# mlvlab/BLiM

Hardware: AMD Instinct MI355X
Metric: candidate-pairs/sec (7B, 96+32 tok) (higher is better)
Workload: dtype f16; 1 GPU; SYN v2t-VTG re-rank: Qwen2-7B dims (28 layers), seeded synthetic weights, 96 video + 32 text tokens per pair, top-16 text candidates per video query, 55 queries (880 pairs, 32560 packed tokens, 28160 label rows) per step per GPU; prefix_reuse=True, vtg_compensated=none, parallelism=query rows sharded over 1 GPU(s); RCCL all-gather of score rows at the end

## Files before the change

blim_amd/csrc/gemm.hip:

```cpp
#include "gemm.hpp"
#include "kernels.hpp"
#include <type_traits>

#define BM 256
#define BN 256
#define BK 64
#define NTHREADS 512
#define TILE_BYTES (BM * BK * 2)
#define BUF_BYTES (2 * TILE_BYTES)
#define GROUP_M 8

typedef const __attribute__((address_space(1))) void* gptr_t;
typedef __attribute__((address_space(3))) void* lptr_t;

__device__ __forceinline__ void glds16(const void* g, char* lds_wave_base) {
    __builtin_amdgcn_global_load_lds((gptr_t)g, (lptr_t)lds_wave_base, 16, 0, 0);
}

__device__ __forceinline__ float gelu_erf(float x) {
    const float z = fabsf(x) * 0.70710678118654752f;
    const float t = __builtin_amdgcn_rcpf(fmaf(0.3275911f, z, 1.0f));
    const float poly = t * fmaf(t, fmaf(t, fmaf(t, fmaf(t, 1.061405429f, -1.453152027f), 1.421413741f), -0.284496736f), 0.254829592f);
    const float erf_abs = 1.0f - poly * __expf(-z * z);
    return 0.5f * x * (1.0f + copysignf(erf_abs, x));
}
__device__ __forceinline__ float silu_f(float x) { return x * __builtin_amdgcn_rcpf(1.0f + __expf(-x)); }

template <int EPI, int DT, bool SPLIT = false, bool MXA = false>
__global__ __launch_bounds__(NTHREADS) void gemm_kernel(const GemmParams p) {
    __shared__ __attribute__((aligned(16))) char smem[5 * TILE_BYTES];

    constexpr bool LO6_BF16_FENCE = MXA && DT == DT_BF16;
    const int tid = threadIdx.x;
    const int lane = tid & 63;
    const int wave = __builtin_amdgcn_readfirstlane(tid >> 6);
    const int wm = wave >> 2, wn = wave & 3;
    int stamp_vb = blockIdx.x;
    auto stamp = [&](int k) __attribute__((always_inline)) {
        if (p.debug_stamps && tid == 0) p.debug_stamps[(size_t)stamp_vb * 8 + k] = __builtin_amdgcn_s_memrealtime();
    };
    const int ntm = (p.M + BM - 1) / BM, ntn = (p.N + BN - 1) / BN;
    const int nwg = ntm * ntn;
#pragma unroll 1
    for (int vb = blockIdx.x; vb < (p.tile_map ? ((nwg + 255) & ~255) : nwg); vb += gridDim.x) {
    int pid;
    if (p.tile_map) {
        const int xcd = vb & 7, k = vb >> 3;
        pid = ((k >> 5) * 8 + xcd) * 32 + (k & 31);
        if (pid >= nwg) continue;
    } else {
        const int bid = vb, xcd = bid & 7, q = nwg >> 3, r = nwg & 7;
        pid = (xcd < r ? xcd * (q + 1) : r * (q + 1) + (xcd - r) * q) + (bid >> 3);
    }
    stamp_vb = pid;
    stamp(0);
    if constexpr (out16<DT>::value == DT_F16 || (LO6_BF16_FENCE)) { if (p.f16_saturate) f16_saturate_off(); }
    const int width = p.group_m * ntn;
    const int first_m = (pid / width) * p.group_m;
    const int gsz = min(ntm - first_m, p.group_m);
    const int tm = first_m + (pid % width) % gsz;
    const int tn = (pid % width) / gsz;
    const int row0 = tm * BM, col0 = tn * BN;

    const int sr = lane >> 3;
    const char* baseA = (const char*)p.A;
    const char* baseW = (const char*)p.W;

    constexpr int ES = (DT == DT_F8) ? 1 : 2;
    constexpr bool MX8 = MXA && DT == DT_F8;
    constexpr bool LO6 = MXA && DT != DT_F8;
    constexpr int ODT = out16<DT>::value;
    const int fr = lane & 15, fc = lane >> 4;
    const int fg = (fr >> 1) & 7;
    const int frag_off = (fr >> 3) * 1024 + (fr & 7) * 128 + 16 * ((fc ^ (fg & 3)) + 4 * (fg >> 2));
    const int a_off = (16 * wm) * 1024 + frag_off;
    const int b_off = (8 * wn) * 1024 + frag_off;

    f32x4 acc[8][4];
#pragma unroll
    for (int i = 0; i < 8; ++i)
#pragma unroll
        for (int j = 0; j < 4; ++j) acc[i][j] = (f32x4){0.f, 0.f, 0.f, 0.f};

    const int nk = p.K * ES / (BK * 2);
    const int nk6 = LO6 ? p.K6 / 128 : 0;
    float f8_scale = 0.f;
    if constexpr (DT == DT_F8) f8_scale = tid < 256 ? (p.row_scale ? p.row_scale[min(row0 + tid, p.M - 1)] : 1.0f) : p.col_scale[min(col0 + tid - 256, p.N - 1)];
    stamp(1);
    {
        const int grp = wave >> 2;
        typedef int i32x8 __attribute__((ext_vector_type(8)));
        typedef int i32x4 __attribute__((ext_vector_type(4)));
        bf16x8 fa[2][8], fb[2][4];
        i32x8 fa8[8], fb8[4];
        auto load_frags = [&](int offA_tile, int offB_tile) __attribute__((always_inline)) {
            const char* ba[2] = {smem + (offA_tile + a_off), smem + ((offA_tile + a_off) ^ 64)};
            const char* bb[2] = {smem + (offB_tile + b_off), smem + ((offB_tile + b_off) ^ 64)};
            if constexpr (DT == DT_F8) {
                auto rd = [](const char* q0, const char* q1) __attribute__((always_inline)) {
                    const i32x4 l = *(const i32x4*)q0, h = *(const i32x4*)q1;
                    return (i32x8){l[0], l[1], l[2], l[3], h[0], h[1], h[2], h[3]};
                };
#pragma unroll
                for (int ni = 0; ni < 4; ++ni) fb8[ni] = rd(bb[0] + ni * 2048, bb[1] + ni * 2048);
#pragma unroll
                for (int mi = 0; mi < 8; ++mi) fa8[mi] = rd(ba[0] + mi * 2048, ba[1] + mi * 2048);
            } else {
#pragma unroll
                for (int ks = 0; ks < 2; ++ks) {
#pragma unroll
                    for (int ni = 0; ni < 4; ++ni) fb[ks][ni] = *(const bf16x8*)(bb[ks] + ni * 2048);
#pragma unroll
                    for (int mi = 0; mi < 8; ++mi) fa[ks][mi] = *(const bf16x8*)(ba[ks] + mi * 2048);
                }
            }
        };
        uint2 mx_cur = make_uint2(0x7f7f7f7fu, 0x7f7f7f7fu), mx_nxt = mx_cur;
        const uint8_t* mx_base = nullptr;
        if constexpr (MX8) {
            int frm = fr;
            asm volatile("" : "+v"(frm));
            mx_base = p.a_mx + (int64_t)tm * 256 + (wm * 16 + frm) * 8;
        }
        auto mx_request = [&](int kt) __attribute__((always_inline)) {
            if constexpr (MX8) mx_nxt = *(const uint2*)(mx_base + (int64_t)min(kt, nk - 1) * p.mx_stride);
        };
        auto compute = [&]() __attribute__((always_inline)) {
            __builtin_amdgcn_s_setprio(1);
            if constexpr (DT == DT_F8) {
#define F8_ROW(MI)                                                                                                                                  \
                _Pragma("unroll") for (int ni = 0; ni < 4; ++ni)                                                                                    \
                    acc[MI][ni] = __builtin_amdgcn_mfma_scale_f32_16x16x128_f8f6f4(fb8[ni], fa8[MI], acc[MI][ni], 0, 0, 0, 0x7f7f7f7f, (MX8 ? (MI & 3) : 0), \
                                                                                  (int)(MX8 ? ((MI) < 4 ? mx_cur.x : mx_cur.y) : 0x7f7f7f7fu));
                F8_ROW(0) F8_ROW(1) F8_ROW(2) F8_ROW(3) F8_ROW(4) F8_ROW(5) F8_ROW(6) F8_ROW(7)
#undef F8_ROW
            } else {
#pragma unroll
                for (int ks = 0; ks < 2; ++ks)
#pragma unroll
                    for (int mi = 0; mi < 8; ++mi)
#pragma unroll
                        for (int ni = 0; ni < 4; ++ni)
                            acc[mi][ni] = mfma16<DT>(fb[ks][ni], fa[ks][mi], acc[mi][ni]);
            }
// ... 966 lines not shown
    if constexpr (ODT == DT_F16) { if (p.f16_saturate) f16_saturate_off(); }

    const int wrow0 = row0 + 32 * wm, wcol0 = col0 + 32 * wn;
    const int tq = lane >> 4, rsub = lane & 15;
    const bool rotated = wcol0 < p.rope_cols;
    float4 qkv_bias[2];
#pragma unroll
    for (int ni = 0; ni < 2; ++ni) {
        const int col = wcol0 + 16 * ni + 4 * tq;
        qkv_bias[ni] = col + 3 < p.N ? *(const float4*)(p.bias + col) : make_float4(0.f, 0.f, 0.f, 0.f);
    }
    const int g = (wcol0 & 127) >> 5;
    float4 cs[2], sn[2];
#pragma unroll
    for (int mi = 0; mi < 2; ++mi) cs[mi] = sn[mi] = make_float4(0.f, 0.f, 0.f, 0.f);
    if (rotated) {
        const int64_t cstride = p.rope_stride * 16;
#pragma unroll
        for (int mi = 0; mi < 2; ++mi) {
            const int row = min(wrow0 + 16 * mi + rsub, p.M - 1);
            const float* base = p.rope_rows + (int64_t)row * 16 + 4 * tq;
            cs[mi] = *(const float4*)(base + g * cstride);
            sn[mi] = *(const float4*)(base + (4 + g) * cstride);
        }
    }

    const NarrowAcc walked = narrow_walk<DT, LO6>(p, tm, tn, lane, wave);
    const f32x4 (&acc)[2][2] = walked.v;

    if constexpr (ODT == DT_F16) { if (p.f16_saturate) f16_saturate_on(); }
    auto ST = [&](int row, int col, float a_, float b_, float c_, float d_) __attribute__((always_inline)) {
        const uint2 hi_ = make_uint2(pack2<ODT>(a_, b_), pack2<ODT>(c_, d_));
        uint2 lo_ = make_uint2(0u, 0u);
        if constexpr (SPLIT) {
            const uint16_t* h16_ = (const uint16_t*)&hi_;
            lo_ = make_uint2(pack2<ODT>(a_ - from16<ODT>(h16_[0]), b_ - from16<ODT>(h16_[1])), pack2<ODT>(c_ - from16<ODT>(h16_[2]), d_ - from16<ODT>(h16_[3])));
        }
        if (row >= p.M || col + 3 >= p.N) return;
        bf16_t* out = (bf16_t*)p.C + (int64_t)row * p.ldc + col;
        *(uint2*)out = hi_;
        if constexpr (SPLIT) *(uint2*)(out + p.lo_off) = lo_;
    };
    if (rotated) {
        const int ncol = (wcol0 & ~127) + 16 * g + 4 * tq;
#pragma unroll
        for (int mi = 0; mi < 2; ++mi) {
            const int row = wrow0 + 16 * mi + rsub;
            const float4 c = cs[mi], sv = sn[mi];
            const float c4[4] = {c.x, c.y, c.z, c.w}, s4[4] = {sv.x, sv.y, sv.z, sv.w};
            const float4 b0 = qkv_bias[0], b1 = qkv_bias[1];
            const float bl[4] = {b0.x, b0.y, b0.z, b0.w}, bh[4] = {b1.x, b1.y, b1.z, b1.w};
            float lo[4], hi[4];
#pragma unroll
            for (int j = 0; j < 4; ++j) {
                const float x1 = acc[mi][0][j] + bl[j];
                const float x2 = acc[mi][1][j] + bh[j];
                lo[j] = __builtin_fmaf(x1, c4[j], -__fmul_rn(x2, s4[j]));
                hi[j] = __builtin_fmaf(x2, c4[j], __fmul_rn(x1, s4[j]));
            }
            ST(row, ncol, lo[0], lo[1], lo[2], lo[3]);
            ST(row, ncol + 64, hi[0], hi[1], hi[2], hi[3]);
        }
    } else {
#pragma unroll
        for (int mi = 0; mi < 2; ++mi) {
            const int row = wrow0 + 16 * mi + rsub;
#pragma unroll
            for (int ni = 0; ni < 2; ++ni) {
                const float4 bv = qkv_bias[ni];
                ST(row, wcol0 + 16 * ni + 4 * tq, acc[mi][ni][0] + bv.x, acc[mi][ni][1] + bv.y, acc[mi][ni][2] + bv.z, acc[mi][ni][3] + bv.w);
            }
        }
    }
}

#include <stdlib.h>
#include <algorithm>
#include <atomic>
static int g_gemm_skip_epi = getenv("BLIM_GEMM_SKIP_EPI") ? atoi(getenv("BLIM_GEMM_SKIP_EPI")) : 0;
static unsigned long long* g_gemm_stamps = nullptr;
static int g_stamp_epi = getenv("BLIM_GEMM_STAMP_EPI") ? atoi(getenv("BLIM_GEMM_STAMP_EPI")) : -1;
static int g_stamp_k = getenv("BLIM_GEMM_STAMP_K") ? atoi(getenv("BLIM_GEMM_STAMP_K")) : -1;
void gemm_set_debug_stamps(unsigned long long* buf) { g_gemm_stamps = buf; }

template <int EPI>
static int launch_t(const GemmParams& p, hipStream_t stream) {
    const int ntm = (p.M + BM - 1) / BM, ntn = (p.N + BN - 1) / BN;
    static int n_cu = 0;
    if (n_cu == 0) {
        int dev = 0;
        if (hipGetDevice(&dev) != hipSuccess || hipDeviceGetAttribute(&n_cu, hipDeviceAttributeMultiprocessorCount, dev) != hipSuccess || n_cu <= 0) n_cu = 256;
        n_cu = (n_cu / 8) * 8;
        if (n_cu < 8) n_cu = 8;
    }
    const dim3 grid(ntm * ntn < n_cu ? ntm * ntn : n_cu);
    void (*kernel)(const GemmParams) = nullptr;
    if constexpr (EPI == EPI_QKV || EPI == EPI_SWIGLU || EPI == EPI_RESID || EPI == EPI_LSE) {
        if (p.A6) {
#define LO6_KERNEL(DTX)                                                                                    \
            if constexpr (EPI == EPI_RESID || EPI == EPI_LSE) kernel = gemm_kernel<EPI, DTX, false, true>; \
            else if (p.lo_off != 0) kernel = gemm_kernel<EPI, DTX, true, true>;                            \
            else if constexpr (EPI == EPI_SWIGLU) kernel = gemm_kernel<EPI, DTX, false, true>;             \
            else { blim_set_error("lo6 QKV GEMM: hi | lo outputs only"); return BLIM_ERR_ARG; }
            if (p.dtype == DT_F16) { LO6_KERNEL(DT_F16) } else { LO6_KERNEL(DT_BF16) }
#undef LO6_KERNEL
        }
    }
    if constexpr (EPI == EPI_BF16 || EPI == EPI_QKV || EPI == EPI_SWIGLU) {
        if (!kernel && p.lo_off != 0) {
            if (p.dtype == DT_F16) kernel = gemm_kernel<EPI, DT_F16, true>;
            else if (p.dtype == DT_BF16) kernel = gemm_kernel<EPI, DT_BF16, true>;
            else { blim_set_error("split (hi|lo) GEMM outputs need a 16-bit engine"); return BLIM_ERR_ARG; }
        }
    }
    if constexpr (EPI == EPI_RESID) {
        if (!kernel && p.dtype == DT_F8 && p.a_mx) kernel = gemm_kernel<EPI, DT_F8, false, true>;
    }
    if (!kernel) {
        if (p.dtype == DT_F8) kernel = gemm_kernel<EPI, DT_F8>;
        else if (p.dtype == DT_F16) kernel = gemm_kernel<EPI, DT_F16>;
        else kernel = gemm_kernel<EPI, DT_BF16>;
    }
    hipLaunchKernelGGL(kernel, grid, dim3(NTHREADS), 0, stream, p);
    hipError_t e = hipGetLastError();
    if (e != hipSuccess) {
        blim_set_error("gemm launch failed: %s", hipGetErrorString(e));
        return BLIM_ERR_HIP;
    }
    return BLIM_OK;
}

static int launch_one(GemmEpi epi, const GemmParams& p_in, hipStream_t stream);

static bool narrow_eligible(GemmEpi epi, const GemmParams& p) {
    return epi == EPI_RESID && (p.dtype == DT_F16 || p.dtype == DT_BF16) && !p.A6 && !p.W6 && !p.a_mx && !p.swiglu_act && !p.debug_stamps && !p.debug_skip_epilogue;
}
static bool narrow_lo6_eligible(GemmEpi epi, const GemmParams& p) {
    return epi == EPI_RESID && (p.dtype == DT_F16 || p.dtype == DT_BF16) && p.A6 && p.W6 && p.w_wrap_k == 0 && !p.a_mx && !p.swiglu_act && !p.debug_stamps && !p.debug_skip_epilogue;
}
static bool narrow_qkv_eligible(GemmEpi epi, const GemmParams& p) {
    return epi == EPI_QKV && (p.dtype == DT_F16 || p.dtype == DT_BF16) && !(p.A6 && p.lo_off == 0) && p.lo_off % 4 == 0 && !p.a_mx && !p.debug_stamps && !p.debug_skip_epilogue;
}
#define NARROW_LAUNCH(...) hipLaunchKernelGGL((__VA_ARGS__), grid, dim3(N_THREADS), 0, stream, p)
static void launch_narrow(const GemmParams& p, dim3 grid, hipStream_t stream) {
    if (p.dtype == DT_F16) NARROW_LAUNCH(gemm_narrow_kernel<DT_F16>); else NARROW_LAUNCH(gemm_narrow_kernel<DT_BF16>);
}
static void launch_narrow_lo6(const GemmParams& p, dim3 grid, hipStream_t stream) {
    if (p.dtype == DT_F16) NARROW_LAUNCH(gemm_narrow_lo6_kernel<DT_F16>); else NARROW_LAUNCH(gemm_narrow_lo6_kernel<DT_BF16>);
}
template <int DT>
static void launch_narrow_qkv_t(const GemmParams& p, dim3 grid, hipStream_t stream) {
    if (p.A6) NARROW_LAUNCH(gemm_nqkv_kernel<DT, true, true>);
    else if (p.lo_off != 0) NARROW_LAUNCH(gemm_nqkv_kernel<DT, true, false>);
    else NARROW_LAUNCH(gemm_nqkv_kernel<DT, false, false>);
}
static void launch_narrow_qkv(const GemmParams& p, dim3 grid, hipStream_t stream) {
    if (p.dtype == DT_F16) launch_narrow_qkv_t<DT_F16>(p, grid, stream); else launch_narrow_qkv_t<DT_BF16>(p, grid, stream);
}
#undef NARROW_LAUNCH
struct NarrowForm {
    int GemmParams::*field;
    const char* name;
    const char* kernel;
    const char* tag;
    bool (*eligible)(GemmEpi, const GemmParams&);
    int threshold;
    void (*launch)(const GemmParams&, dim3, hipStream_t);
    std::atomic<int64_t> launches;
};
static NarrowForm g_narrow_forms[3] = {
    {&GemmParams::narrow, "narrow", "the narrow kernel", "narrow", narrow_eligible, GEMM_NARROW_TILES, launch_narrow, {0}},
    {&GemmParams::narrow_lo6, "narrow_lo6", "the narrow e2m3 kernel", "narrow lo6", narrow_lo6_eligible, GEMM_NARROW_LO6_TILES, launch_narrow_lo6, {0}},
    {&GemmParams::narrow_qkv, "narrow_qkv", "the narrow QKV kernel", "narrow qkv", narrow_qkv_eligible, GEMM_NARROW_QKV_TILES, launch_narrow_qkv, {0}},
};
extern "C" int64_t blim_gemm_narrow_launches(void) { return g_narrow_forms[0].launches.load(); }
extern "C" int32_t blim_gemm_narrow_threshold(void) { return g_narrow_forms[0].threshold; }
extern "C" int64_t blim_gemm_narrow_lo6_launches(void) { return g_narrow_forms[1].launches.load(); }
extern "C" int32_t blim_gemm_narrow_lo6_threshold(void) { return g_narrow_forms[1].threshold; }
extern "C" int64_t blim_gemm_narrow_qkv_launches(void) { return g_narrow_forms[2].launches.load(); }
extern "C" int32_t blim_gemm_narrow_qkv_threshold(void) { return g_narrow_forms[2].threshold; }
static NarrowForm* narrow_chosen(GemmEpi epi, const GemmParams& p) {
    for (NarrowForm& f : g_narrow_forms) {
        const int v = p.*f.field;
        if (v == 0 || !f.eligible(epi, p)) continue;
        if (v == 2 || (int64_t)((p.M + BM - 1) / BM) * ((p.N + BN - 1) / BN) < f.threshold) return &f;
    }
    return nullptr;
}
static int launch_narrow_form(NarrowForm& f, const GemmParams& p, hipStream_t stream) {
    f.launch(p, dim3((unsigned)(((p.M + NBM - 1) / NBM) * ((p.N + NBN - 1) / NBN))), stream);
    hipError_t e = hipGetLastError();
    if (e != hipSuccess) { blim_set_error("%s gemm launch failed: %s", f.tag, hipGetErrorString(e)); return BLIM_ERR_HIP; }
    f.launches.fetch_add(1);
    return BLIM_OK;
}

int launch_gemm(GemmEpi epi, const GemmParams& p, hipStream_t stream) {
    ARG_CHECK(p.M > 0 && p.N > 0 && p.K > 0 && p.lda > 0);
    ARG_CHECK(p.dtype == DT_BF16 || p.dtype == DT_F16 || p.dtype == DT_F8);
    const int64_t es = p.dtype == DT_F8 ? 1 : 2;
    const int64_t row_bytes = p.lda * es;
    if ((int64_t)p.M * row_bytes < (1ll << 32)) return launch_one(epi, p, stream);
    const int64_t chunk = ((1ll << 32) - 1) / row_bytes / BM * BM;
    ARG_CHECK(chunk >= BM);
    const int64_t c_es = (epi == EPI_F32 || epi == EPI_RESID) ? 4 : 2;
    const int ntn = (p.N + BN - 1) / BN;
    for (int64_t r0 = 0; r0 < p.M; r0 += chunk) {
        GemmParams q = p;
        q.M = (int)std::min<int64_t>(chunk, p.M - r0);
        q.A = (const bf16_t*)((const char*)p.A + r0 * row_bytes);
        if (p.C) q.C = (char*)p.C + r0 * p.ldc * c_es;
        if (p.row_scale) q.row_scale = p.row_scale + r0;
        if (p.rope_rows) q.rope_rows = p.rope_rows + r0 * 16;
        if (p.a_mx) q.a_mx = p.a_mx + r0;
        if (p.out_mx) q.out_mx = p.out_mx + r0;
        if (p.A6) q.A6 = p.A6 + (r0 / BM) * (int64_t)(p.K6 / 128) * F6_TILE_BYTES;
        if (p.out6) q.out6 = p.out6 + (r0 / BM) * (int64_t)(p.N / BN) * F6_TILE_BYTES;
        if (p.labels) q.labels = p.labels + r0;
        if (p.lse_part) q.lse_part = p.lse_part + r0 * ntn;
        if (p.label_logit) q.label_logit = p.label_logit + r0;
        if (p.resid_in) q.resid_in = p.resid_in + r0 * p.ldc;
        if (p.swiglu_gu) q.swiglu_gu = p.swiglu_gu + r0 * p.swiglu_ld;
        if (p.swiglu_act) q.swiglu_act = p.swiglu_act + r0 * p.swiglu_act_ld;
        const int rc = launch_one(epi, q, stream);
        if (rc != BLIM_OK) return rc;
    }
    return BLIM_OK;
}

static int launch_one(GemmEpi epi, const GemmParams& p_in, hipStream_t stream) {
    GemmParams p = p_in;
    p.debug_skip_epilogue = g_gemm_skip_epi;
    p.group_m = GROUP_M;
    const int64_t n_tiles = (int64_t)((p.M + BM - 1) / BM) * ((p.N + BN - 1) / BN);
    p.tile_map = ((p.N + BN - 1) / BN <= 32 && n_tiles >= 256) ? 1 : 0;
    p.debug_stamps = ((g_stamp_epi < 0 || g_stamp_epi == (int)epi) && (g_stamp_k < 0 || g_stamp_k == p.K)) ? g_gemm_stamps : nullptr;
    ARG_CHECK(p.M > 0 && p.N > 0 && p.K > 0);
    ARG_CHECK(p.A && p.W);
    ARG_CHECK(p.dtype == DT_BF16 || p.dtype == DT_F16 || p.dtype == DT_F8);
    const int es = p.dtype == DT_F8 ? 1 : 2;
    ARG_CHECK((int64_t)p.K * es % 128 == 0);
    ARG_CHECK(p.lda * es % 16 == 0);
    ARG_CHECK(p.dtype != DT_F8 || ((p.row_scale || p.a_mx) && p.col_scale));
    ARG_CHECK((!p.a_mx && !p.out_mx) || (p.dtype == DT_F8 && p.mx_stride >= (int64_t)((p.M + BM - 1) / BM) * 256));
    ARG_CHECK(!p.a_mx || epi == EPI_RESID);
    ARG_CHECK(!p.A6 || ((p.dtype == DT_F16 || p.dtype == DT_BF16) && p.W6 && p.w_wrap_k == 0 && p.K6 > 0 && p.K6 % 128 == 0 && (epi == EPI_RESID || epi == EPI_QKV || epi == EPI_SWIGLU || epi == EPI_LSE)));
    ARG_CHECK(!p.out_mx || (epi == EPI_SWIGLU && p.N % 256 == 0 && p.ldc % 16 == 0));
    ARG_CHECK(!p.out6 || (epi == EPI_SWIGLU && p.A6 && p.lo_off > 0 && p.N % 256 == 0));
    ARG_CHECK(p.w_wrap_k == 0 || (p.K == 2 * p.w_wrap_k && (int64_t)p.w_wrap_k * es % 128 == 0));
    ARG_CHECK(p.lo_off == 0 || epi == EPI_BF16 || epi == EPI_QKV || epi == EPI_SWIGLU);
    for (const NarrowForm& f : g_narrow_forms)
        if (p.*f.field < 0 || p.*f.field > 2) { blim_set_error("gemm: %s = %d (0 = the 256 x 256 kernel, 1 = auto, 2 = %s wherever it is eligible)", f.name, p.*f.field, f.kernel); return BLIM_ERR_ARG; }
    ARG_CHECK((int64_t)p.M * p.lda * es < (1ll << 32) && (int64_t)p.N * (p.w_wrap_k > 0 ? p.w_wrap_k : p.K) * es < (1ll << 32));
    switch (epi) {
        case EPI_BF16:
            ARG_CHECK(p.C && p.ldc % 4 == 0);
            ARG_CHECK(!p.swiglu_gu || (p.N % 16 == 0 && p.swiglu_ld % 8 == 0 && p.swiglu_ld >= 2 * (int64_t)p.N));
            ARG_CHECK(!p.swiglu_act || (p.N % 32 == 0 && p.swiglu_act_ld % 8 == 0 && p.swiglu_act_ld >= p.N / 2 && !p.swiglu_gu));
            return launch_t<EPI_BF16>(p, stream);
        case EPI_F32: ARG_CHECK(p.C && p.bias == nullptr); return launch_t<EPI_F32>(p, stream);
        case EPI_RESID:
            ARG_CHECK(p.C && p.ldc % 4 == 0);
            if (NarrowForm* f = narrow_chosen(epi, p)) return launch_narrow_form(*f, p, stream);
            return launch_t<EPI_RESID>(p, stream);
        case EPI_QKV:
            ARG_CHECK(p.C && p.bias && p.rope_rows && p.rope_stride >= p.M && p.N % 128 == 0 && p.rope_cols % 128 == 0 && p.ldc % 4 == 0);
            if (NarrowForm* f = narrow_chosen(epi, p)) return launch_narrow_form(*f, p, stream);
            return launch_t<EPI_QKV>(p, stream);
        case EPI_SWIGLU: ARG_CHECK(p.C && p.N % 32 == 0 && p.ldc % 4 == 0); return launch_t<EPI_SWIGLU>(p, stream);
        case EPI_LSE: ARG_CHECK(p.labels && p.lse_part && p.label_logit); return launch_t<EPI_LSE>(p, stream);
    }
    blim_set_error("unknown epilogue %d", (int)epi);
    return BLIM_ERR_ARG;
}
```

blim_amd/csrc/gemm.hpp:

```cpp
#pragma once
#include "common.hpp"

enum GemmEpi : int {
    EPI_BF16 = 0,
    EPI_F32 = 1,
    EPI_RESID = 2,
    EPI_QKV = 3,
    EPI_SWIGLU = 4,
    EPI_LSE = 5,
};

struct GemmParams {
    int dtype;
    const float* row_scale;
    const float* col_scale;
    const bf16_t* A;
    int64_t lda;
    const bf16_t* W;
    int M, N, K;
    void* C;
    int64_t ldc;
    const float* bias;
    const float* resid_in;
    uint16_t* swiglu_gu;
    int64_t swiglu_ld;
    uint16_t* swiglu_act;
    int64_t swiglu_act_ld;
    int act;
    float scale;
    int rope_cols;
    const float* rope_rows;
    int64_t rope_stride;
    const int32_t* labels;
    float2* lse_part;
    float* label_logit;
    int w_wrap_k;
    int64_t lo_off;
    uint8_t* out_mx;
    const uint8_t* a_mx;
    int64_t mx_stride;
    const uint8_t* A6;
    const uint8_t* W6;
    int K6;
    uint8_t* out6;
    int f16_saturate;
    int group_m;
    int tile_map;
    int debug_skip_epilogue;
    unsigned long long* debug_stamps;
    int narrow;
    int narrow_lo6;
    int narrow_qkv;
};
#define GEMM_NARROW_TILES 57
#define GEMM_NARROW_LO6_TILES 57
#define GEMM_NARROW_QKV_TILES 55
void gemm_set_debug_stamps(unsigned long long* buf);

int launch_gemm(GemmEpi epi, const GemmParams& p, hipStream_t stream);

static inline int qkv_perm_row(int cprime) { return 16 * (cprime >> 5) + (cprime & 15) + 64 * ((cprime >> 4) & 1); }
```

blim_amd/engine.py:

```python
from __future__ import annotations

import ctypes as C
import os
import re
from typing import Dict, List, Optional, Sequence

import numpy as np

from .synth import ModelDims, weight_shapes

_HERE = os.path.dirname(os.path.abspath(__file__))
LIB_PATH = os.environ.get("BLIM_LIB_PATH") or os.path.join(_HERE, "libblim_hip.so")
HEADER_PATH = os.path.join(os.path.dirname(_HERE), "include", "blim.h")

DTYPE_F32, DTYPE_BF16 = 0, 1
COMPUTE_DTYPES = {"bf16": 0, "f16": 1, "f8": 2}
DEFAULT_COMPUTE_DTYPE = os.environ.get("BLIM_DTYPE", "f16")


def torch_dtype_of(name: str):
    import torch
    return {"bf16": torch.bfloat16, "f16": torch.float16, "f8": torch.float16}[name]


# ... 103 lines not shown
    vp, i32, i64, u64, f32 = C.c_void_p, C.c_int32, C.c_int64, C.c_uint64, C.c_float
    sig = {
        "blim_abi_version": ([], C.c_int),
        "blim_last_error": ([], C.c_char_p),
        "blim_create": ([C.POINTER(Config), C.POINTER(vp)], C.c_int),
        "blim_destroy": ([vp], None),
        "blim_load_weight": ([vp, C.c_char_p, vp, i32, i32], C.c_int),
        "blim_init_synthetic_weights": ([vp, u64], C.c_int),
        "blim_weights_ready": ([vp], C.c_int),
        "blim_load_adapter": ([vp, C.c_char_p, vp, vp, i32, f32], C.c_int),
        "blim_clear_adapters": ([vp], C.c_int),
        "blim_num_adapters": ([vp], C.c_int),
        "blim_reserve": ([vp, i64, i64], C.c_int),
        "blim_project_video": ([vp, vp, i64, i32, vp, vp], C.c_int),
        "blim_group_mean": ([vp, vp, i64, i32, vp, vp], C.c_int),
        "blim_assemble": ([vp, vp, i64, vp, vp, vp], C.c_int),
        "blim_decode": ([vp, C.POINTER(Batch), vp, vp, i64, vp, vp, vp], C.c_int),
        "blim_vtg_logprobs": ([vp, vp, vp, i64, vp, vp], C.c_int),
        "blim_segment_mean": ([vp, vp, vp, i32, i32, vp, vp], C.c_int),
        "blim_lm_head": ([vp, vp, i64, vp, vp], C.c_int),
        "blim_ce_rows": ([vp, vp, i64, i32, vp, i64, vp, vp], C.c_int),
        "blim_visual_head": ([vp, vp, i64, vp, vp], C.c_int),
        "blim_visual_head_f32": ([vp, vp, i64, vp, vp], C.c_int),
        "blim_tvg_scores": ([vp, vp, vp, i32, vp, i32, vp, vp], C.c_int),
        "blim_tvg_logits": ([vp, vp, vp, i32, i32, vp, vp], C.c_int),
        "blim_set_video_vocab": ([vp, vp, i32, vp], C.c_int),
        "blim_tvg_logits_f32": ([vp, vp, i32, vp, vp], C.c_int),
        "blim_score_vtg": ([vp, C.POINTER(Batch), vp, vp, vp, i64, vp, i32, vp, vp], C.c_int),
        "blim_score_tvg": ([vp, C.POINTER(Batch), vp, vp, vp, i32, vp, i32, vp, vp], C.c_int),
        "blim_forward": ([vp, vp, vp, i32, i32, vp, vp, vp], C.c_int),
        "blim_fill_bell_bf16": ([vp, i64, u64, C.c_char_p, f32, f32, vp], C.c_int),
        "blim_fill_bell_f32": ([vp, i64, u64, C.c_char_p, f32, f32, i32, vp], C.c_int),
        "blim_gemm_bf16": ([vp, i64, vp, i32, i32, i32, vp, i64, vp], C.c_int),
        "blim_gemm_f16": ([vp, i64, vp, i32, i32, i32, vp, i64, vp], C.c_int),
        "blim_f6_tiles_bytes": ([i64, i32], C.c_int64),
        "blim_gemm_f16_lo6": ([vp, vp, i32, i32, i32, vp, vp, vp, vp], C.c_int),
        "blim_quant_rows": ([vp, i64, i64, i32, i32, vp, vp, vp], C.c_int),
        "blim_gemm_f8": ([vp, i64, vp, vp, vp, i32, i32, i32, vp, i64, vp], C.c_int),
        "blim_attention": ([C.POINTER(AttentionArgs), vp], C.c_int),
        "blim_attention_bwd_workspace_bytes": ([i64, i32, i32, i32], C.c_int64),
        "blim_attention_bwd": ([C.POINTER(AttentionBwdArgs), vp], C.c_int),
        "blim_rope_bwd": ([vp, vp, i64, i32, i32, vp, vp, vp, i32, i32, vp], C.c_int),
        "blim_lora_down_workspace_bytes": ([i32, i32], C.c_int64),
        "blim_lora_down": ([C.POINTER(LoraDownArgs), vp], C.c_int),
        "blim_lora_grads_workspace_bytes": ([i32, i64, i32, i32, i32], C.c_int64),
        "blim_lora_grads": ([C.POINTER(LoraGradsArgs), vp], C.c_int),
        "blim_lora_dx": ([C.POINTER(LoraDxArgs), vp], C.c_int),
        "blim_rmsnorm_bwd": ([C.POINTER(RmsnormBwdArgs), vp], C.c_int),
        "blim_ce_workspace_bytes": ([i64], C.c_int64),
        "blim_ce_fwd_bwd": ([vp, i64, i32, vp, i32, i64, f32, vp, vp, i64, vp, i32, vp, i64, vp], C.c_int),
        "blim_gelu": ([i32, vp, i64, vp, vp, i64, i32, i32, vp], C.c_int),
        "blim_adamw_raw": ([vp, vp, vp, vp, i64, f32, f32, f32, f32, f32, f32, i32, vp], C.c_int),
        "blim_grad_stats_workspace_bytes": ([i64], C.c_int64),
        "blim_grad_stats_raw": ([vp, i64, f32, vp, vp, i64, vp], C.c_int),
        "blim_rmsnorm": ([C.POINTER(RmsnormArgs), vp], C.c_int),
        "blim_rmsnorm_f8": ([vp, i64, i64, i32, vp, f32, vp, vp, vp], C.c_int),
        "blim_lse_combine": ([vp, i32, vp, vp, i64, vp, vp], C.c_int),
        "blim_tvg_criterion": ([vp, i64, i32, vp, i32, i32, vp, vp], C.c_int),
        "blim_tvg_rank": ([vp, i64, i32, i32, vp, i64, i32, vp, f32, i32, vp, vp, vp, i64, vp], C.c_int),
        "blim_tvg_rank_within": ([vp, i64, i32, i32, vp, i64, i32, i32, vp, vp, vp, vp, i32, f32, i32, vp, vp, vp], C.c_int),
        "blim_rank_rows": ([vp, i64, i32, i32, i32, vp, vp, vp], C.c_int),
        "blim_tvg_cols": ([vp, i64, i32, i32, vp, i32, vp, i64, i64, vp], C.c_int),
        "blim_score_tvg_first": ([vp, C.POINTER(Batch), vp, vp, i32, vp, i32, vp, f32, i32, vp, vp, vp, vp], C.c_int),
        "blim_score_tvg_first_within": ([vp, C.POINTER(Batch), vp, vp, i32, vp, i32, i32, vp, vp, vp, vp, i32, f32, i32, vp, vp, vp], C.c_int),
        "blim_tvg_first_cached": ([vp, vp, vp, i32, vp, i32, vp, i64, i32, vp], C.c_int),
        "blim_group_mean_rows": ([vp, vp, i64, i32, i32, i32, i32, vp], C.c_int),
        "blim_assemble_rows": ([vp, vp, i64, i32, vp, vp, i32, vp], C.c_int),
        "blim_gemm": ([C.POINTER(GemmArgs), vp], C.c_int),
        "blim_gemm_narrow_launches": ([], C.c_int64),
        "blim_gemm_narrow_threshold": ([], C.c_int32),
        "blim_gemm_narrow_lo6_launches": ([], C.c_int64),
        "blim_gemm_narrow_lo6_threshold": ([], C.c_int32),
        "blim_gemm_narrow_qkv_launches": ([], C.c_int64),
        "blim_gemm_narrow_qkv_threshold": ([], C.c_int32),
        "blim_rope_rows_bytes": ([i32], C.c_int64),
        "blim_rope_rows": ([vp, i64, f32, i32, vp, vp, i64, vp], C.c_int),
        "blim_timing_enable": ([vp, i32], C.c_int),
        "blim_timing_num_classes": ([], C.c_int),
        "blim_timing_class_name": ([i32], C.c_char_p),
        "blim_timing_report": ([vp, C.POINTER(C.c_double), C.POINTER(C.c_int64), C.POINTER(C.c_double)], C.c_int),
        "blim_set_option": ([vp, C.c_char_p, i32], C.c_int),
        "blim_debug_read": ([vp, C.c_char_p, vp, i64, vp], C.c_int),
        "blim_debug_gemm_stamps": ([vp], C.c_int),
        "blim_hash_device": ([vp, i64, vp, vp], C.c_int),
        "blim_weights_fingerprint": ([vp, vp, vp], C.c_int),
        "blim_prefix_cache_bytes": ([vp, i32, i32, i32], C.c_int64),
        "blim_prefix_cache_create": ([vp, i32, i32, i32, C.POINTER(vp)], C.c_int),
        "blim_prefix_cache_destroy": ([vp], None),
        "blim_prefix_cache_fill": ([vp, vp, C.POINTER(Batch), vp, vp, vp], C.c_int),
        "blim_prefix_cache_slot_len": ([vp, i32], C.c_int),
        "blim_score_vtg_cached": ([vp, vp, C.POINTER(Batch), vp, vp, i32, vp, vp, vp, i64, vp, i32, vp, vp], C.c_int),
        "blim_score_tvg_cached": ([vp, vp, C.POINTER(Batch), vp, vp, i32, vp, vp, vp, i32, vp, i32, vp, vp], C.c_int),
        "blim_score_vtg_admit": ([vp, vp, C.POINTER(Batch), vp, vp, i32, vp, i32, vp, vp, vp, i64, vp, i32, vp, vp], C.c_int),
        "blim_score_tvg_admit": ([vp, vp, C.POINTER(Batch), vp, vp, i32, vp, i32, vp, vp, vp, i32, vp, i32, vp, vp], C.c_int),
        "blim_prefix_cache_record_bytes": ([vp, i32], C.c_int64),
        "blim_prefix_cache_export": ([vp, vp, vp, i32, vp, i64, vp, vp], C.c_int),
        "blim_prefix_cache_import": ([vp, vp, vp, i32, vp, i64, vp, vp], C.c_int),
    }
    for name, (args, res) in sig.items():
        fn = getattr(lib, name)
        fn.argtypes = args
        fn.restype = res
    _lib = lib
    return lib


def _check(rc: int, what: str):
    if rc != 0:
        raise BlimError(f"{what} failed (code {rc}): {load_library().blim_last_error().decode()}")


def _ptr(t) -> int:
    if t is None:
        return None
    assert t.is_cuda and t.is_contiguous(), "engine buffers must be contiguous device tensors"
    return t.data_ptr()


def _stream() -> int:
    import torch
    return torch.cuda.current_stream().cuda_stream


def vocab_key_of(video_vocab):
    if not hasattr(video_vocab, "data_ptr"):
        return (id(video_vocab),)
    flat = video_vocab.reshape(-1)
    pick = flat[:: max(1, flat.numel() // 4096)][:4096].double()
    fp = (float(pick.sum()), float((pick * pick).sum()))
    return (video_vocab.data_ptr(), tuple(video_vocab.shape), int(getattr(video_vocab, "_version", 0)), fp)


class PackedBatch:

    def __init__(self, positions: np.ndarray, key_visible: np.ndarray, seq_start: np.ndarray, seq_len: np.ndarray,
                 pfx_start: Optional[np.ndarray] = None, pfx_len: Optional[np.ndarray] = None, device="cuda", own_start: Optional[np.ndarray] = None):
        import torch
        n_seqs = len(seq_start)
        if pfx_start is None:
            pfx_start = np.zeros(n_seqs, dtype=np.int32)
            pfx_len = np.zeros(n_seqs, dtype=np.int32)
        seq_len = np.asarray(seq_len, dtype=np.int32)
        nblk = (seq_len + 31) // 32
        blk_seq = np.repeat(np.arange(n_seqs, dtype=np.int32), nblk)
        blk_q0 = (np.concatenate([np.arange(n, dtype=np.int32) for n in nblk]) * 32).astype(np.int32) if n_seqs else np.zeros(0, np.int32)
        self.n_tokens = int(len(positions))
        self.max_position = int(np.max(positions)) if len(positions) else 0
        self.n_seqs = int(n_seqs)
        self.n_blocks = int(len(blk_seq))
        parts = [np.asarray(positions, np.int32), np.asarray(seq_start, np.int32), seq_len, np.asarray(pfx_start, np.int32),
                 np.asarray(pfx_len, np.int32), blk_seq, blk_q0]
        offs = np.cumsum([0] + [len(p) for p in parts])
        flat = torch.from_numpy(np.concatenate(parts)).to(device)
        self._flat = flat
        self.positions, self.seq_start, self.seq_len, self.pfx_start, self.pfx_len, self.blk_seq, self.blk_q0 = \
            [flat[offs[i]:offs[i + 1]] for i in range(7)]
        self.key_visible = torch.from_numpy(np.ascontiguousarray(key_visible, dtype=np.uint8)).to(device)
        self.own_start = None
        if own_start is not None and np.any(np.asarray(own_start) != 0):
            own_start = np.asarray(own_start, dtype=np.int32)
            assert len(own_start) == self.n_tokens
            self.own_start = torch.from_numpy(np.ascontiguousarray(own_start)).to(device)

    def struct(self, max_positions: Optional[int] = None) -> Batch:
        if max_positions is not None and self.max_position >= max_positions:
            raise BlimError(f"a sequence reaches position {self.max_position} but the engine's RoPE table holds {max_positions} positions: "
# ... 752 lines not shown
```

include/blim.h:

```cpp
#ifndef BLIM_H_
#define BLIM_H_
#include <stdint.h>
#ifdef __cplusplus
extern "C" {
#endif

#define BLIM_ABI_VERSION 9
#define BLIM_ERR_ARG (-1)
#define BLIM_ERR_HIP (-2)
#define BLIM_ERR_STATE (-3)
#define BLIM_ERR_NOMEM (-4)

#define BLIM_DTYPE_F32 0
#define BLIM_DTYPE_BF16 1

#define BLIM_COMPUTE_BF16 0
#define BLIM_COMPUTE_F16 1
#define BLIM_COMPUTE_F8 2

typedef struct blim_engine blim_engine;

typedef struct blim_config {
    int32_t vocab_size, hidden_size, intermediate_size, num_layers, num_heads, num_kv_heads;
    int32_t mm_hidden_size;
// ... 280 lines not shown
int blim_rmsnorm(const blim_rmsnorm_args* args, void* stream);
int blim_rmsnorm_f8(const float* x, int64_t ldx, int64_t n_rows, int32_t H, const float* w, float eps, void* out8, float* scale, void* stream);
int blim_lse_combine(const float* part, int32_t n_tiles, const float* label_logit, const int32_t* labels, int64_t n_rows, float* logprob, void* stream);
int blim_tvg_criterion(const float* logits, int64_t ld, int32_t n_vocab, const int32_t* labels, int32_t n_pairs, int32_t clips, float* score, void* stream);
#define BLIM_TVG_RANK_MAX_K 1024
int blim_tvg_rank(const float* logits, int64_t ld, int32_t n_vocab, int32_t n_rows, const float* prior_logits, int64_t ld_prior, int32_t n_prior,
                  const int32_t* prior_of, float alpha, int32_t k, int32_t* idx_out, float* val_out, float* logprob_out, int64_t ld_out, void* stream);
int blim_tvg_rank_within(const float* logits, int64_t ld, int32_t n_vocab, int32_t n_rows, const float* prior_logits, int64_t ld_prior, int32_t n_prior, int32_t n_q,
                         const int32_t* row_of, const int32_t* prior_of, const int32_t* within, const int32_t* within_off, int32_t n_within, float alpha, int32_t k,
                         int32_t* idx_out, float* val_out, void* stream);
int blim_rank_rows(const float* values, int64_t ld, int32_t n, int32_t n_rows, int32_t k, int32_t* idx_out, float* val_out, void* stream);
int blim_tvg_cols(const float* logits, int64_t ld, int32_t n_vocab, int32_t n_rows, const int32_t* cols, int32_t n_cols, float* out, int64_t ld_out, int64_t out0,
                  void* stream);
int blim_group_mean_rows(void* out, const void* in, int64_t n_out, int32_t group, int32_t H, int32_t dtype16, int32_t split, void* stream);
int blim_assemble_rows(void* out, const int32_t* src_index, int64_t n_tokens, int32_t H, const void* table, const void* feats, int32_t split, void* stream);

#define BLIM_EPI_BF16 0
#define BLIM_EPI_F32 1
#define BLIM_EPI_RESID 2
#define BLIM_EPI_QKV 3
#define BLIM_EPI_SWIGLU 4
#define BLIM_EPI_LSE 5
typedef struct blim_gemm_args {
    int64_t struct_bytes;
    int32_t epi;
    int32_t dtype;
    const void* A;
    int64_t lda;
    const void* W;
    int32_t M, N, K;
    int32_t act;
    void* C;
    int64_t ldc;
    const float* bias;
    const float* resid_in;
    float scale;
    int32_t w_wrap_k;
    int64_t lo_off;
    int32_t f16_saturate;
    int32_t rope_cols;
    const float* rope_rows;
    int64_t rope_stride;
    const int32_t* labels;
    float* lse_part;
    float* label_logit;
    const float* row_scale;
    const float* col_scale;
    const void* a_mx;
    void* out8;
    void* out_mx;
    int64_t mx_stride;
    void* A6;
    void* W6;
    int32_t K6;
    int32_t f6_build;
    void* out6;
    void* swiglu_act;
    int64_t swiglu_act_ld;
    void* swiglu_gu;
    int64_t swiglu_ld;
    int32_t tile;
    int32_t tile_lo6;
    int32_t tile_qkv;
} blim_gemm_args;
int blim_gemm(const blim_gemm_args* args, void* stream);
int64_t blim_gemm_narrow_launches(void);
int32_t blim_gemm_narrow_threshold(void);
int64_t blim_gemm_narrow_lo6_launches(void);
int32_t blim_gemm_narrow_lo6_threshold(void);
int64_t blim_gemm_narrow_qkv_launches(void);
int32_t blim_gemm_narrow_qkv_threshold(void);
int64_t blim_rope_rows_bytes(int32_t max_positions);
int blim_rope_rows(const int32_t* positions, int64_t n_tokens, float rope_theta, int32_t max_positions, void* workspace, float* out, int64_t stride, void* stream);

int blim_timing_enable(blim_engine* e, int32_t on);
int blim_timing_num_classes(void);
const char* blim_timing_class_name(int32_t cls);
int blim_timing_report(blim_engine* e, double* ms, int64_t* calls, double* flops);

int blim_debug_read(blim_engine* e, const char* which, void* dst, int64_t bytes, void* stream);

int blim_debug_gemm_stamps(void* device_buf);

int blim_set_option(blim_engine* e, const char* key, int32_t value);

typedef struct blim_vision blim_vision;
typedef struct blim_vision_config {
    int32_t image_size;
    int32_t patch_size;
    int32_t num_frames;
    int32_t hidden_size;
    int32_t num_heads;
    int32_t mlp_hidden;
    int32_t depth;
    int32_t tome_tokens;
    int32_t compute_dtype;
} blim_vision_config;
int blim_vision_create(const blim_vision_config* cfg, blim_vision** out);
void blim_vision_destroy(blim_vision* v);
int blim_vision_load_weight(blim_vision* v, const char* name, const void* data, int32_t dtype, int32_t on_device);
int blim_vision_init_synthetic_weights(blim_vision* v, uint64_t seed);
int blim_vision_set_pos_embed(blim_vision* v, const float* table_host);
int blim_vision_ready(const blim_vision* v);
int blim_vision_encode(blim_vision* v, const void* frames, int32_t n_clips, float* out_feat, float* out_tome, void* stream);
int blim_vit_attention(const void* qkv, int32_t n_clips, int32_t L, int32_t heads, int32_t dtype16, void* out, void* stream);
int blim_tome_merge(blim_vision* v, const float* x, int32_t b, int32_t p, int32_t c, int32_t heads, int32_t target, float* out, void* stream);

int64_t blim_preprocess_workspace_bytes(int32_t T, int32_t H, int32_t W, int32_t S);
int blim_preprocess_frames(const uint8_t* frames,
                           int32_t T, int32_t H, int32_t W, int32_t S,
                           const int32_t* xb, const int32_t* xk, int32_t xks,
                           const int32_t* yb, const int32_t* yk, int32_t yks,
                           const uint16_t* lut,
                           void* out,
                           void* workspace, void* stream);

typedef struct blim_trainer blim_trainer;
typedef struct blim_train_config {
    int32_t lora_r;
    float lora_alpha;
    float lora_dropout;
} blim_train_config;
int64_t blim_train_flat_size(const blim_engine* e, int32_t lora_r);
int blim_train_param_offset(const blim_engine* e, int32_t lora_r, const char* name, int64_t* offset, int64_t* rows, int64_t* cols);
int blim_train_create(blim_engine* e, const blim_train_config* cfg, float* params, float* grads, blim_trainer** out);
void blim_train_destroy(blim_trainer* t);
int blim_train_sync_params(blim_trainer* t, void* stream);
int blim_train_merge(blim_trainer* t, void* stream);
typedef struct blim_train_batch {
    const blim_batch* batch;
    const int32_t* src_index;
    const void* feats;
    int64_t n_feat_rows;
    int32_t tok_per_clip;
    int32_t max_seq_len;
    const int32_t* rows;
    const int32_t* labels;
    int64_t n_rows;
    const int32_t* tvg_rows;
    const int32_t* tvg_labels;
    int64_t n_tvg_rows;
    const void* vocab;
    int32_t n_vocab;
    float grad_scale;
    uint64_t dropout_seed;
} blim_train_batch;
int blim_train_step(blim_trainer* t, const blim_train_batch* b, float* loss_sums, void* stream);
int blim_train_grad_stats(blim_trainer* t, float inv_scale, float* stats, void* stream);
int blim_train_adamw(blim_trainer* t, float* exp_avg, float* exp_avg_sq, float lr, float beta1, float beta2, float eps, float weight_decay, float inv_scale,
                     int32_t step, void* stream);
int blim_train_debug_read(blim_trainer* t, const char* which, void* dst, int64_t bytes, void* stream);

#ifdef __cplusplus
}
#endif
#endif
```

Baseline: 2683 pairs/s.

## Add column-lockstep tile ordering for wide LSE (lm-head) GEMMs

Adds a third tile map for the LSE-epilogue GEMM when N is wide (more than 32 column tiles). Work-groups on each XCD are assigned tiles in bands of rows and groups of four columns, so concurrently running tiles share weight columns and A rows in cache. The band height is picked from the row-tile count. It also adds debug hooks to force a tile map and to dump the ordering. The risk is a worse ordering or load imbalance for some shapes, plus extra index arithmetic per tile.

Result: no change. 2687 pairs/s (median of 2 runs) (+0.2%).

```diff
diff --git a/blim_amd/csrc/gemm.hip b/blim_amd/csrc/gemm.hip
--- a/blim_amd/csrc/gemm.hip
+++ b/blim_amd/csrc/gemm.hip
@@ -43,8 +43,12 @@
     const int nwg = ntm * ntn;
 #pragma unroll 1
     for (int vb = blockIdx.x; vb < (p.tile_map ? ((nwg + 255) & ~255) : nwg); vb += gridDim.x) {
-    int pid;
-    if (p.tile_map) {
+    int pid, tm, tn;
+    constexpr bool LOCKSTEP = EPI == EPI_LSE;
+    if (LOCKSTEP && p.tile_map == 2) {
+        if (!tile_of_lockstep(vb, ntm, ntn, p.group_m, &tm, &tn, &pid)) continue;
+        pid = tm * ntn + tn;
+    } else if (p.tile_map) {
         const int xcd = vb & 7, k = vb >> 3;
         pid = ((k >> 5) * 8 + xcd) * 32 + (k & 31);
         if (pid >= nwg) continue;
@@ -55,11 +59,13 @@
     stamp_vb = pid;
     stamp(0);
     if constexpr (out16<DT>::value == DT_F16 || (LO6_BF16_FENCE)) { if (p.f16_saturate) f16_saturate_off(); }
-    const int width = p.group_m * ntn;
-    const int first_m = (pid / width) * p.group_m;
-    const int gsz = min(ntm - first_m, p.group_m);
-    const int tm = first_m + (pid % width) % gsz;
-    const int tn = (pid % width) / gsz;
+    if (!LOCKSTEP || p.tile_map != 2) {
+        const int width = p.group_m * ntn;
+        const int first_m = (pid / width) * p.group_m;
+        const int gsz = min(ntm - first_m, p.group_m);
+        tm = first_m + (pid % width) % gsz;
+        tn = (pid % width) / gsz;
+    }
     const int row0 = tm * BM, col0 = tn * BN;
 
     const int sr = lane >> 3;
@@ -1192,6 +1198,33 @@
 static int g_stamp_epi = getenv("BLIM_GEMM_STAMP_EPI") ? atoi(getenv("BLIM_GEMM_STAMP_EPI")) : -1;
 static int g_stamp_k = getenv("BLIM_GEMM_STAMP_K") ? atoi(getenv("BLIM_GEMM_STAMP_K")) : -1;
 void gemm_set_debug_stamps(unsigned long long* buf) { g_gemm_stamps = buf; }
+static std::atomic<int> g_tile_map_force{-1};
+extern "C" int blim_debug_gemm_tile_map(int32_t map) {
+    if (map < -1 || map > 2) { blim_set_error("gemm: tile map %d (-1 = by shape, 0 = XCD chunks, 1 = round-robin groups, 2 = column lockstep)", (int)map); return BLIM_ERR_ARG; }
+    g_tile_map_force.store(map);
+    return BLIM_OK;
+}
+static std::atomic<int> g_tile_map_last{-1};
+extern "C" int32_t blim_gemm_last_tile_map(void) { return g_tile_map_last.load(); }
+static int tile_map_for(GemmEpi epi, int ntm, int ntn) {
+    const int64_t n_tiles = (int64_t)ntm * ntn;
+    if (ntn <= 32) return n_tiles >= 256 ? 1 : 0;
+    if (ntm <= GROUP_M || epi != EPI_LSE) return 0;
+    const int64_t band = (int64_t)GROUP_M * ntn;
+    return (n_tiles % 8 == 0 && (n_tiles / 8) % band == 0) ? 0 : 2;
+}
+extern "C" int64_t blim_gemm_lockstep_order(int32_t ntm, int32_t ntn, int32_t* tile_of_vb, int64_t capacity, int32_t* map_by_shape) {
+    if (ntm <= 0 || ntn <= 0 || (int64_t)ntm * ntn > (1ll << 30) || !tile_of_vb) return -1;
+    const int64_t n_vb = ((int64_t)ntm * ntn + 255) & ~255ll;
+    if (capacity < n_vb) return -1;
+    const int band_m = lockstep_band_m(ntm);
+    for (int64_t vb = 0; vb < n_vb; ++vb) {
+        int tm = 0, tn = 0, pos = 0;
+        tile_of_vb[vb] = tile_of_lockstep((int)vb, ntm, ntn, band_m, &tm, &tn, &pos) ? tm * ntn + tn : -1;
+    }
+    if (map_by_shape) *map_by_shape = tile_map_for(EPI_LSE, ntm, ntn);
+    return n_vb;
+}
 
 template <int EPI>
 static int launch_t(const GemmParams& p, hipStream_t stream) {
@@ -1342,8 +1375,10 @@
     GemmParams p = p_in;
     p.debug_skip_epilogue = g_gemm_skip_epi;
     p.group_m = GROUP_M;
-    const int64_t n_tiles = (int64_t)((p.M + BM - 1) / BM) * ((p.N + BN - 1) / BN);
-    p.tile_map = ((p.N + BN - 1) / BN <= 32 && n_tiles >= 256) ? 1 : 0;
+    const int force = g_tile_map_force.load();
+    p.tile_map = (force >= 0 && !(force == 2 && epi != EPI_LSE)) ? force : tile_map_for(epi, (p.M + BM - 1) / BM, (p.N + BN - 1) / BN);
+    g_tile_map_last.store(p.tile_map);
+    if (p.tile_map == 2 && !narrow_chosen(epi, p)) p.group_m = lockstep_band_m((p.M + BM - 1) / BM);
     p.debug_stamps = ((g_stamp_epi < 0 || g_stamp_epi == (int)epi) && (g_stamp_k < 0 || g_stamp_k == p.K)) ? g_gemm_stamps : nullptr;
     ARG_CHECK(p.M > 0 && p.N > 0 && p.K > 0);
     ARG_CHECK(p.A && p.W);
diff --git a/blim_amd/csrc/gemm.hpp b/blim_amd/csrc/gemm.hpp
--- a/blim_amd/csrc/gemm.hpp
+++ b/blim_amd/csrc/gemm.hpp
@@ -52,6 +52,37 @@
     int narrow_lo6;
     int narrow_qkv;
 };
+static inline int lockstep_band_m(int ntm) {
+    const int s = (ntm + 63) / 64;
+    return ((ntm + s - 1) / s + 7) / 8 * 8;
+}
+#if defined(__HIPCC__) || defined(__CUDACC__)
+#define GEMM_HD __host__ __device__
+#else
+#define GEMM_HD
+#endif
+GEMM_HD static inline bool tile_of_lockstep(int vb, int ntm, int ntn, int band_m, int* tm, int* tn, int* pos_out) {
+    const int nwg = ntm * ntn;
+    const int xcd = vb & 7, k = vb >> 3, w = k >> 5, i = k & 31;
+    const int nfull = nwg >> 8;
+    int pos;
+    if (w < nfull) pos = (w << 8) + (xcd << 5) + i;
+    else {
+        const int n = nwg & 255, lo = (xcd * n) >> 3, hi = ((xcd + 1) * n) >> 3;
+        if (w > nfull || i >= hi - lo) return false;
+        pos = (nfull << 8) + lo + i;
+    }
+    const int sbw = band_m * ntn, s = pos / sbw, q = pos - s * sbw;
+    const int r0 = s * band_m, hs = ntm - r0 < band_m ? ntm - r0 : band_m;
+    const int cg = q / (hs * 4), q2 = q - cg * (hs * 4);
+    const int cw = ntn - 4 * cg < 4 ? ntn - 4 * cg : 4;
+    const int rb = q2 / (8 * cw), q3 = q2 - rb * (8 * cw);
+    const int bh = hs - 8 * rb < 8 ? hs - 8 * rb : 8;
+    *tm = r0 + 8 * rb + q3 % bh;
+    *tn = 4 * cg + q3 / bh;
+    *pos_out = pos;
+    return true;
+}
 #define GEMM_NARROW_TILES 57
 #define GEMM_NARROW_LO6_TILES 57
 #define GEMM_NARROW_QKV_TILES 55
diff --git a/blim_amd/engine.py b/blim_amd/engine.py
--- a/blim_amd/engine.py
+++ b/blim_amd/engine.py
@@ -209,6 +209,9 @@
         "blim_set_option": ([vp, C.c_char_p, i32], C.c_int),
         "blim_debug_read": ([vp, C.c_char_p, vp, i64, vp], C.c_int),
         "blim_debug_gemm_stamps": ([vp], C.c_int),
+        "blim_debug_gemm_tile_map": ([i32], C.c_int),
+        "blim_gemm_last_tile_map": ([], C.c_int32),
+        "blim_gemm_lockstep_order": ([i32, i32, vp, i64, vp], C.c_int64),
         "blim_hash_device": ([vp, i64, vp, vp], C.c_int),
         "blim_weights_fingerprint": ([vp, vp, vp], C.c_int),
         "blim_prefix_cache_bytes": ([vp, i32, i32, i32], C.c_int64),
diff --git a/include/blim.h b/include/blim.h
--- a/include/blim.h
+++ b/include/blim.h
@@ -386,6 +386,10 @@
 
 int blim_debug_gemm_stamps(void* device_buf);
 
+int blim_debug_gemm_tile_map(int32_t map);
+int32_t blim_gemm_last_tile_map(void);
+int64_t blim_gemm_lockstep_order(int32_t ntm, int32_t ntn, int32_t* tile_of_vb, int64_t capacity, int32_t* map_by_shape);
+
 int blim_set_option(blim_engine* e, const char* key, int32_t value);
 
 typedef struct blim_vision blim_vision;
```
